# juniorliu95/replication_faster_rcnn

Measured on AMD Instinct MI355X. Metric: images/sec through RPN proposal+NMS+RoIPool; RoIPool HBM GB/s vs peak, higher is better.
Workload: dtype fp32; 1 GPU; cfg2: 8 images/GPU, VOC shape 600x1000, 38x63x9 anchors, 6000->300 NMS@0.7, RoIPool 7x7x256; global_batch=8, images_per_gpu=8, parallelism=dp1 (per-image sharding), streams=2, prop_streams=4, pool_on=prop, rng_waits=front, roi_cg=auto, roi_split=auto, roi_store=auto, prop_cus=0, devices=1, hw_queues=8

## Files before the change

### replication_faster_rcnn_amd/csrc/capi.cpp

```cpp
#include <hip/hip_runtime.h>

#include <cstdarg>
#include <cstdio>
#include <cstdlib>
#include <atomic>
#include <cstring>
#include <mutex>

#include "common.h"

namespace frcnn {

static thread_local char g_err[512] = "";
constexpr int kMaxDevices = 64;

void set_error(const char* fmt, ...) {
    va_list ap;
    va_start(ap, fmt);
    vsnprintf(g_err, sizeof(g_err), fmt, ap);
    va_end(ap);
}

int check_launch(const char* what) {
    hipError_t e = hipGetLastError();
    if (e != hipSuccess) {
        set_error("%s: %s", what, hipGetErrorString(e));
        return FRCNN_EHIP;
    }
    return FRCNN_OK;
}

static PathCfg g_path;

const PathCfg& path_cfg() { return g_path; }

int device_cu_count() {
    static std::atomic<int> cus[kMaxDevices] = {};
    int dev = 0;
    if (hipGetDevice(&dev) != hipSuccess || dev < 0 || dev >= kMaxDevices) {
        (void)hipGetLastError();
        return 256;
    }
    int n = cus[dev].load(std::memory_order_relaxed);
    if (n <= 0) {
        if (hipDeviceGetAttribute(&n, hipDeviceAttributeMultiprocessorCount, dev) != hipSuccess || n <= 0) {
            (void)hipGetLastError();
            n = 256;
        }
        cus[dev].store(n, std::memory_order_relaxed);
    }
    return n;
}

}

extern "C" const char* frcnn_version(void) { return "frcnn_mi355x 0.2.0 gfx950"; }

extern "C" int frcnn_set_path(const char* op, const char* path) {
    using namespace frcnn;
    if (!op || !path) {
        set_error("frcnn_set_path: null argument");
        return FRCNN_EINVAL;
    }
    auto is = [&](const char* a, const char* b) { return std::strcmp(a, b) == 0; };
    const bool aut = is(path, "auto");
    if (is(op, "roi_pool_fwd") &&
        (aut || is(path, "wave") || is(path, "dense") || is(path, "generic"))) {
        g_path.roi_fwd = aut ? kPathAuto : is(path, "generic") ? kPathGeneric
                                       : is(path, "dense")     ? kPathDense
                                                               : kPathWave;
    } else if (is(op, "roi_pool_bwd") &&
               (aut || is(path, "ring") || is(path, "plain"))) {
        g_path.roi_bwd = aut ? kPathAuto : is(path, "plain") ? kPathPlain : kPathRing;
    } else if (is(op, "propose") &&
               (aut || is(path, "hybrid") || is(path, "lazy") || is(path, "wide"))) {
        g_path.propose = aut ? kPathAuto : is(path, "hybrid") ? kPathHybrid
                                         : is(path, "lazy")   ? kPathLazy
                                                              : kPathWide;
    } else if (is(op, "roi_pool_fwd_store") && (aut || is(path, "temporal") || is(path, "nt"))) {
        g_path.roi_store = is(path, "nt") ? 1 : 0;
    } else if (is(op, "sampler") && (aut || is(path, "walk") || is(path, "chip") || is(path, "chip_only") ||
                                     is(path, "chip_tight"))) {
        g_path.sampler = aut                   ? kPathAuto
                         : is(path, "walk")      ? kPathWalk
                         : is(path, "chip")      ? kPathChip
                         : is(path, "chip_only") ? kPathChipOnly
                                                 : kPathChipTight;
    } else if (is(op, "roi_pool_split")) {
        char* end = nullptr;
        const long v = aut ? 0 : std::strtol(path, &end, 10);
        if (!aut && (end == path || *end != '\0' || v < 0 || v > 64)) {
            set_error("frcnn_set_path: roi_pool_split must be auto or 0..64, got '%s'", path);
            return FRCNN_EINVAL;
        }
        g_path.roi_split = static_cast<int>(v);
    } else if (is(op, "roi_pool_cg") && (aut || is(path, "4") || is(path, "8") || is(path, "16"))) {
        g_path.roi_cg = aut ? 0 : std::atoi(path);
    } else {
        set_error("frcnn_set_path: unknown op / path '%s' / '%s'", op, path);
        return FRCNN_EINVAL;
    }
    return FRCNN_OK;
}

extern "C" const char* frcnn_last_error(void) { return frcnn::g_err; }

extern "C" int frcnn_device_cu_count(int* out) {
    int dev = 0, n = 0;
    if (!out) {
        frcnn::set_error("frcnn_device_cu_count: null pointer");
        return FRCNN_EINVAL;
    }
    if (hipGetDevice(&dev) != hipSuccess ||
        hipDeviceGetAttribute(&n, hipDeviceAttributeMultiprocessorCount, dev) != hipSuccess)
        return frcnn::check_launch("frcnn_device_cu_count");
    *out = n;
    return FRCNN_OK;
}

extern "C" int frcnn_stream_create(const uint32_t* cu_mask, int words, void** out) {
    if (!out || words < 0 || (words > 0 && !cu_mask)) {
        frcnn::set_error("frcnn_stream_create: bad arguments");
        return FRCNN_EINVAL;
    }
    hipStream_t s = nullptr;
    const hipError_t e = words > 0 ? hipExtStreamCreateWithCUMask(&s, static_cast<uint32_t>(words), cu_mask)
                                   : hipStreamCreateWithFlags(&s, hipStreamNonBlocking);
    if (e != hipSuccess) {
        frcnn::set_error("frcnn_stream_create: %s", hipGetErrorString(e));
        return FRCNN_EHIP;
    }
    *out = s;
    return FRCNN_OK;
}

namespace frcnn {
struct CuCache {
    std::mutex mu;
    hipStream_t s[16] = {};
    int dev[16] = {};
    int n[16] = {};
    int next = 0;
};
static CuCache g_cu_cache;

static void cu_cache_evict(hipStream_t st) {
    std::lock_guard<std::mutex> lk(g_cu_cache.mu);
    for (int i = 0; i < 16; ++i)
        if (g_cu_cache.s[i] == st) g_cu_cache.s[i] = nullptr;
}
}

extern "C" int frcnn_stream_destroy(void* stream) {
    if (!stream) return FRCNN_OK;
    frcnn::cu_cache_evict(frcnn::as_stream(stream));
    if (hipStreamDestroy(frcnn::as_stream(stream)) != hipSuccess)
        return frcnn::check_launch("frcnn_stream_destroy");
    return FRCNN_OK;
}

namespace frcnn {
int stream_cu_count(hipStream_t s) {
    const int all = device_cu_count();
// ... 55 lines not shown
```

### replication_faster_rcnn_amd/csrc/common.h

```cpp
#pragma once

#include <hip/hip_runtime.h>

#include <cstdint>
#include <cstdio>
#include <string>

#include "../../include/frcnn_capi.h"

namespace frcnn {

void set_error(const char* fmt, ...);

constexpr int kPathAuto = 0;
constexpr int kPathGeneric = 1;
constexpr int kPathDense = 2;
constexpr int kPathWave = 3;
constexpr int kPathPlain = 1;
constexpr int kPathRing = 2;
constexpr int kPathHybrid = 1;
constexpr int kPathLazy = 2;
constexpr int kPathWide = 3;
constexpr int kPathWalk = 1;
constexpr int kPathChip = 2;
constexpr int kPathChipOnly = 3;
constexpr int kPathChipTight = 4;
struct PathCfg {
    int roi_fwd = kPathAuto;
    int roi_bwd = kPathAuto;
    int propose = kPathAuto;
    int roi_split = 0;
    int roi_cg = 0;
    int sampler = kPathAuto;
    int roi_store = 0;
};
const PathCfg& path_cfg();

int device_cu_count();
int stream_cu_count(hipStream_t s);

int check_launch(const char* what);

#define FRCNN_REQUIRE(cond, ...)                 \
    do {                                         \
        if (!(cond)) {                           \
            ::frcnn::set_error(__VA_ARGS__);     \
            return FRCNN_EINVAL;                 \
        }                                        \
    } while (0)

#define FRCNN_LAUNCH_CHECK(name)                         \
    do {                                                 \
        int _rc = ::frcnn::check_launch(name);           \
        if (_rc) return _rc;                             \
    } while (0)

inline hipStream_t as_stream(void* s) { return reinterpret_cast<hipStream_t>(s); }

inline size_t align_up(size_t x, size_t a) { return (x + a - 1) / a * a; }

struct Carver {
    char* base;
    size_t off = 0;
    explicit Carver(void* p) : base(static_cast<char*>(p)) {}
    template <class T>
    T* take(size_t count) {
        off = align_up(off, 256);
        T* p = reinterpret_cast<T*>(base ? base + off : nullptr);
        off += count * sizeof(T);
        return p;
    }
    size_t used() const { return align_up(off, 256); }
};

constexpr int kWave = 64;

__device__ __forceinline__ int lane_id() { return __lane_id(); }

__device__ __forceinline__ uint64_t readlane_u64(uint64_t v, int l) {
    uint32_t lo = __builtin_amdgcn_readlane(static_cast<uint32_t>(v), l);
    uint32_t hi = __builtin_amdgcn_readlane(static_cast<uint32_t>(v >> 32), l);
    return (static_cast<uint64_t>(hi) << 32) | lo;
}

__device__ __forceinline__ uint64_t wave_or_u64(uint64_t v) {
    for (int o = 32; o > 0; o >>= 1) v |= __shfl_xor(v, o, 64);
    return v;
}

__device__ __forceinline__ uint32_t wave_sum_u32(uint32_t v) {
    for (int o = 32; o > 0; o >>= 1) v += __shfl_xor(v, o, 64);
    return v;
}

__device__ __forceinline__ uint64_t lanemask_lt() {
    int l = lane_id();
    return l == 0 ? 0ull : (~0ull >> (64 - l));
}

__device__ __forceinline__ uint32_t desc_score_key(float s) {
    if (s != s) return 0u;
    uint32_t u = __float_as_uint(s);
    if (u == 0x80000000u) u = 0u;
    uint32_t asc = (u & 0x80000000u) ? ~u : (u | 0x80000000u);
    return ~asc;
}

__device__ __forceinline__ float clamp_nan(float v, float lo, float hi) {
    if (v != v) return v;
    float t = v < lo ? lo : v;
    return t > hi ? hi : t;
}

__device__ __forceinline__ float exp_cr(float v) { return static_cast<float>(exp(static_cast<double>(v))); }

__device__ __forceinline__ float4 decode_box(float4 a, float4 d) {
    float ah = a.z - a.x;
// ... 15 lines not shown
```

### replication_faster_rcnn_amd/csrc/roi_pool.hip

```cpp
#include <cfloat>
#include <cmath>
#include <cstdlib>
#include <cstring>

#include <type_traits>

#include <hip/hip_bf16.h>
#include <hip/hip_fp16.h>

#include "common.h"

namespace frcnn {

__device__ __forceinline__ float ld_f32(const float* p) { return *p; }
__device__ __forceinline__ float ld_f32(const __half* p) { return __half2float(*p); }
__device__ __forceinline__ float ld_f32(const __hip_bfloat16* p) { return __bfloat162float(*p); }
__device__ __forceinline__ __half cvt_elem(float v, const __half*) { return __float2half(v); }
__device__ __forceinline__ __hip_bfloat16 cvt_elem(float v, const __hip_bfloat16*) { return __float2bfloat16(v); }
__device__ __forceinline__ void st_f32(float* p, float v) { *p = v; }
template <class T>
__device__ __forceinline__ void st_f32(T* p, float v) {
    *p = cvt_elem(v, p);
}
__device__ __forceinline__ void st4_f32(float* p, float a, float b, float c, float d) {
    *reinterpret_cast<float4*>(p) = make_float4(a, b, c, d);
}
template <class T>
__device__ __forceinline__ void st4_f32(T* p, float a, float b, float c, float d) {
    struct alignas(8) Quad {
        T v[4];
    };
    static_assert(sizeof(Quad) == sizeof(uint2), "16-bit element types only");
    const Quad q{{cvt_elem(a, p), cvt_elem(b, p), cvt_elem(c, p), cvt_elem(d, p)}};
    *reinterpret_cast<uint2*>(p) = __builtin_bit_cast(uint2, q);
}
__device__ __forceinline__ void st_nt_f32(float* p, float v) { __builtin_nontemporal_store(v, p); }
template <class T>
__device__ __forceinline__ void st_nt_f32(T* p, float v) {
    static_assert(sizeof(T) == 2, "16-bit element types only");
    __builtin_nontemporal_store(__builtin_bit_cast(uint16_t, cvt_elem(v, p)), reinterpret_cast<uint16_t*>(p));
}

constexpr int kMaxBins = 1024;
constexpr int kListPad = 16;
__host__ __device__ constexpr int64_t list_stride(int64_t R) { return R + kListPad; }
constexpr size_t kLdsPerCu = 160 * 1024;

__device__ __forceinline__ int4 roi_bin(const float* roi, float ss, int H, int W, int PH, int PW,
                                        int ph, int pw) {
    int sw = static_cast<int>(roundf(roi[1] * ss));
    int sh = static_cast<int>(roundf(roi[2] * ss));
    int ew = static_cast<int>(roundf(roi[3] * ss));
    int eh = static_cast<int>(roundf(roi[4] * ss));
    int rw = ew - sw + 1;
    int rh = eh - sh + 1;
    rw = rw > 1 ? rw : 1;
    rh = rh > 1 ? rh : 1;
    float bh = static_cast<float>(rh) / static_cast<float>(PH);
    float bw = static_cast<float>(rw) / static_cast<float>(PW);
    int hs = static_cast<int>(floorf(static_cast<float>(ph) * bh)) + sh;
    int ws = static_cast<int>(floorf(static_cast<float>(pw) * bw)) + sw;
    int he = static_cast<int>(ceilf(static_cast<float>(ph + 1) * bh)) + sh;
    int we = static_cast<int>(ceilf(static_cast<float>(pw + 1) * bw)) + sw;
    hs = min(max(hs, 0), H);
    he = min(max(he, 0), H);
    ws = min(max(ws, 0), W);
    we = min(max(we, 0), W);
    return make_int4(hs, he, ws, we);
}

template <class T>
__device__ __forceinline__ void pool_window(const T* __restrict__ plane, int W, int4 g,
                                            float& mv, int& mi) {
    mv = (g.y <= g.x || g.w <= g.z) ? 0.0f : -FLT_MAX;
    mi = -1;
    for (int h = g.x; h < g.y; ++h) {
        const T* row = plane + h * W;
        for (int w = g.z; w < g.w; ++w) {
            float v = ld_f32(&row[w]);
            if (v > mv) {
                mv = v;
                mi = h * W + w;
            }
// ... 420 lines not shown
                const size_t o = (static_cast<size_t>(r) * C + c0) * PHW + k;
#pragma unroll
                for (int c = 0; c < CG; ++c) {
                    const int idx = mi[c] >> 4;
                    float v = mv[c];
                    if (v == 0.0f && idx >= 0)
                        v = reinterpret_cast<const float*>(tb + (c >> 2) * plane_bytes)[idx * 4 + (c & 3)];
                    st_f32(&out[o + static_cast<size_t>(c) * PHW], v);
                    argmax[o + static_cast<size_t>(c) * PHW] = idx;
                }
            }
            f0 = __builtin_amdgcn_readfirstlane(fn);
        }
    }
}

template <int NT, int CG, int FIX, bool HEAD, bool LIST>
__global__ __launch_bounds__(NT) void roi_pool_fwd_dense_kernel(
    const float* __restrict__ x, const float* __restrict__ rois, const int* __restrict__ list,
    const int* __restrict__ cnt, int R, int C, int H, int W, int PH_, int PW_, float ss,
    float* __restrict__ out, int32_t* __restrict__ argmax, int cap, HeadArgs hd) {
    roi_pool_fwd_dense_body<float, NT, CG, FIX, HEAD, LIST>(x, rois, list, cnt, R, C, H, W, PH_, PW_, ss, out,
                                                            argmax, cap, hd);
}

template <class T, int NT, int CG, int FIX, bool HEAD, bool LIST>
__global__ __launch_bounds__(NT) void roi_pool_fwd_dense_kernel_h(
    const T* __restrict__ x, const float* __restrict__ rois, const int* __restrict__ list,
    const int* __restrict__ cnt, int R, int C, int H, int W, int PH_, int PW_, float ss,
    T* __restrict__ out, int32_t* __restrict__ argmax, int cap, HeadArgs hd) {
    roi_pool_fwd_dense_body<T, NT, CG, FIX, HEAD, LIST>(x, rois, list, cnt, R, C, H, W, PH_, PW_, ss, out, argmax,
                                                        cap, hd);
}

#ifdef FRCNN_POOL_PROF
constexpr int kPoolProfSlots = 8192;
__device__ unsigned long long g_pool_prof[kPoolProfSlots][4];
__device__ unsigned int g_pool_prof_rois[kPoolProfSlots];
#define PPROF_T(k)                                                                                  \
    do {                                                                                            \
        const unsigned long long _t = __builtin_amdgcn_s_memrealtime();                             \
        const unsigned _wg = blockIdx.x + gridDim.x * (blockIdx.y + gridDim.y * blockIdx.z);         \
        if (_wg < kPoolProfSlots) {                                                                 \
            if ((k) == 3) {                                                                         \
                if ((threadIdx.x & 63) == 0) atomicMax(&g_pool_prof[_wg][3], _t);                   \
            } else if (threadIdx.x == 0) {                                                          \
                g_pool_prof[_wg][k] = _t;                                                           \
            }                                                                                       \
        }                                                                                           \
    } while (0)
#define PPROF_ROIS(n)                                                                               \
    do {                                                                                            \
        const unsigned _wg = blockIdx.x + gridDim.x * (blockIdx.y + gridDim.y * blockIdx.z);         \
        if (_wg < kPoolProfSlots && threadIdx.x == 0) g_pool_prof_rois[_wg] = (n);                  \
    } while (0)
#else
#define PPROF_T(k) do {} while (0)
#define PPROF_ROIS(n) do {} while (0)
#endif

constexpr int kFixPx = 2400;

typedef float f32x4 __attribute__((ext_vector_type(4)));
typedef __attribute__((address_space(3))) const f32x4 lds_f32x4;

template <int NP, int KPS>
__device__ __forceinline__ void tile_read(uint32_t a, uint32_t ps, f32x4 (&v)[NP]) {
    const uint32_t P = KPS ? static_cast<uint32_t>(KPS) : ps;
    uint32_t a2 = 0;
    if (NP > 2) {
        if (KPS) asm("v_add_u32_e32 %0, %1, %2" : "=v"(a2) : "i"(2 * KPS), "v"(a));
        else a2 = a + 2 * P;
    }
#pragma unroll
    for (int q = 0; q < NP; ++q) {
        const uint32_t o = q < 2 ? a + q * P : a2 + (q - 2) * P;
        v[q] = *reinterpret_cast<lds_f32x4*>(static_cast<size_t>(o));
    }
}

template <class T, int NT, int CG, int FIX, bool HEAD, bool NTS, int KPS>
__device__ __forceinline__ void roi_pool_fwd_wave_body(
    const T* x, const float* rois, int R, int C, int H, int W, int PH_, int PW_,
    float ss, T* out, int32_t* argmax, int geo_cap, HeadArgs hd) {
    const int PH = FIX ? FIX : PH_, PW = FIX ? FIX : PW_;
    constexpr int NP = CG / 4;
    extern __shared__ __attribute__((aligned(16))) float4 q4[];
    char* const t = reinterpret_cast<char*>(q4);
    if ((size_t)(__attribute__((address_space(3))) float4*)q4 != 0) __builtin_trap();
    const int b = blockIdx.z;
    const int c0 = blockIdx.x * CG;
    const int tid = threadIdx.x, lane = tid & 63;
    const int HW = H * W;
    const int HWs = (HW + 16) & ~15;
    const uint32_t PS = KPS ? static_cast<uint32_t>(KPS) : static_cast<uint32_t>(HWs) * 16u;
    int4* s_geo = reinterpret_cast<int4*>(t + NP * PS);
    int* s_red = reinterpret_cast<int*>(s_geo + geo_cap);
    int* s_next = s_red + 2 * (NT / 64);
    const int PHW = PH * PW;
    const int split = gridDim.y, z = blockIdx.y;
    const int N = gridDim.z - 1;
    PPROF_T(0);
    if (b == N) {
        const int2 rg = HEAD ? roi_range_sorted<NT>(hd.inds, R, 0, N, s_red, 1)
                             : roi_range_sorted<NT>(rois, R, 0, N, s_red);
        const int n_lo = rg.x, tot = n_lo + (R - rg.y);
        const int lo = static_cast<int>(static_cast<int64_t>(tot) * z / split);
        const int hi = static_cast<int>(static_cast<int64_t>(tot) * (z + 1) / split);
        if (HEAD && hd.boxes && blockIdx.x == 0)
            for (int t = lo + tid; t < hi; t += NT) {
                const int r = t < n_lo ? t : rg.y + (t - n_lo);
                float bx[5];
                head_box(rois, hd, r, bx);
#pragma unroll
                for (int j = 0; j < 5; ++j) hd.boxes[static_cast<size_t>(r) * 5 + j] = bx[j];
            }
        for (int e = lo * CG * PHW + tid; e < hi * CG * PHW; e += NT) {
            const int t = e / (CG * PHW);
            const int rem = e - t * (CG * PHW);
            const int r = t < n_lo ? t : rg.y + (t - n_lo);
            const size_t o = (static_cast<size_t>(r) * C + c0) * PHW + rem;
            st_f32(&out[o], 0.0f);
            argmax[o] = -1;
        }
        return;
    }
    const int2 rg = HEAD ? roi_range_sorted<NT>(hd.inds, R, b, b + 1, s_red, 1)
                         : roi_range_sorted<NT>(rois, R, b, b + 1, s_red);
    const int rbase = rg.x, nr = rg.y - rg.x;
    PPROF_T(1);
    if (z >= nr) return;
    const int nmine = (nr - z + split - 1) / split;
    PPROF_ROIS(nmine);
    const T* src = x + (static_cast<size_t>(b) * C + c0) * HW;
    if (tid < NP) *reinterpret_cast<float4*>(t + tid * PS + HW * 16) = make_float4(0.f, 0.f, 0.f, 0.f);
    for (int p = tid; p < HW; p += NT) {
        float v[CG];
#pragma unroll
        for (int q = 0; q < CG; ++q) {
            const float e = ld_f32(&src[static_cast<size_t>(q) * HW + p]);
            v[q] = e > -FLT_MAX ? e : -FLT_MAX;
        }
#pragma unroll
        for (int k = 0; k < NP; ++k)
            *reinterpret_cast<float4*>(t + k * PS + p * 16) = make_float4(v[4 * k], v[4 * k + 1], v[4 * k + 2], v[4 * k + 3]);
    }
    const int ph = lane / PW, pw = lane - (lane / PW) * PW;
    const bool act = lane < PHW;
    for (int k0 = 0; k0 < nmine; k0 += geo_cap) {
        const int cn = min(geo_cap, nmine - k0);
        for (int i = tid; i < cn; i += NT) {
            const int r = rbase + z + (k0 + i) * split;
            float bx[5];
            if (HEAD) {
                head_box(rois, hd, r, bx);
                if (hd.boxes && blockIdx.x == 0) {
#pragma unroll
                    for (int j = 0; j < 5; ++j) hd.boxes[static_cast<size_t>(r) * 5 + j] = bx[j];
                }
            } else {
#pragma unroll
                for (int j = 0; j < 5; ++j) bx[j] = rois[static_cast<size_t>(r) * 5 + j];
            }
            const RoiGeom gm = roi_geom(bx, ss, PH, PW);
            s_geo[i] = make_int4(gm.sh, gm.sw, __float_as_int(gm.bh), __float_as_int(gm.bw));
        }
        if (tid == 0) *s_next = 0;
        __syncthreads();
        if (k0 == 0) PPROF_T(2);
        int k = 0;
        if (lane == 0) k = atomicAdd(s_next, 1);
        k = __builtin_amdgcn_readfirstlane(k);
        while (k < cn) {
            int kn = 0;
            if (lane == 0) kn = atomicAdd(s_next, 1);
            const int r = rbase + z + (k0 + k) * split;
            const int4 gq = s_geo[k];
            RoiGeom gm;
            gm.sh = gq.x;
            gm.sw = gq.y;
            gm.bh = __int_as_float(gq.z);
            gm.bw = __int_as_float(gq.w);
            int4 g = geom_bin(gm, H, W, ph, pw);
            if (!act) g = make_int4(0, 0, 0, 0);
            const bool empty = g.y <= g.x || g.w <= g.z;
            float mv[CG];
            int mi[CG];
            {
                const uint32_t a0 = static_cast<uint32_t>(empty ? HW : g.x * W + g.z) * 16u;
                const float thr = empty ? __int_as_float(0x7f800000) : -FLT_MAX;
                f32x4 v[NP];
                tile_read<NP, KPS>(a0, PS, v);
                __builtin_amdgcn_sched_barrier(0);
#pragma unroll
                for (int q = 0; q < NP; ++q) {
                    const float vv[4] = {v[q].x, v[q].y, v[q].z, v[q].w};
#pragma unroll
                    for (int j = 0; j < 4; ++j) {
                        mv[4 * q + j] = vv[j];
                        mi[4 * q + j] = vv[j] > thr ? static_cast<int>(a0) : -1;
                    }
                }
            }
            for (int h = g.x; h < g.y; ++h) {
                const uint32_t rb = static_cast<uint32_t>(h * W) * 16u;
                const uint32_t ae = rb + static_cast<uint32_t>(g.w) * 16u;
                uint32_t a = rb + static_cast<uint32_t>(h == g.x ? g.z + 1 : g.z) * 16u;
                for (; a < ae; a += 16) {
                    f32x4 v[NP];
                    tile_read<NP, KPS>(a, PS, v);
                    __builtin_amdgcn_sched_barrier(0);
#pragma unroll
                    for (int q = 0; q < NP; ++q) {
                        const float vv[4] = {v[q].x, v[q].y, v[q].z, v[q].w};
#pragma unroll
                        for (int j = 0; j < 4; ++j) {
                            if (vv[j] > mv[4 * q + j]) {
                                mv[4 * q + j] = vv[j];
                                mi[4 * q + j] = static_cast<int>(a);
                            }
                        }
                    }
                }
            }
            if (act) {
                const size_t o = (static_cast<size_t>(r) * C + c0) * PHW + lane;
                T* op = out + o;
                int32_t* ap = argmax + o;
                if constexpr (NTS) {
#pragma unroll
                    for (int c = 0; c < CG; ++c) {
                        st_nt_f32(&op[c * PHW], mv[c]);
                        __builtin_nontemporal_store(mi[c] >> 4, ap + c * PHW);
                    }
                } else {
#pragma unroll
                    for (int c = 0; c < CG; ++c) {
                        st_f32(&op[c * PHW], mv[c]);
                        ap[c * PHW] = mi[c] >> 4;
                    }
                }
            }
            k = __builtin_amdgcn_readfirstlane(kn);
        }
        __syncthreads();
    }
    PPROF_T(3);
}

template <int NT, int CG, int FIX, bool HEAD, bool NTS = false, int KPS = 0>
__global__ __launch_bounds__(NT) void roi_pool_fwd_wave_kernel(
    const float* __restrict__ x, const float* __restrict__ rois, int R, int C, int H, int W, int PH_, int PW_,
    float ss, float* __restrict__ out, int32_t* __restrict__ argmax, int geo_cap, HeadArgs hd) {
    roi_pool_fwd_wave_body<float, NT, CG, FIX, HEAD, NTS, KPS>(x, rois, R, C, H, W, PH_, PW_, ss, out, argmax,
                                                               geo_cap, hd);
}

template <class T, int NT, int CG, int FIX, bool HEAD, bool NTS = false, int KPS = 0>
__global__ __launch_bounds__(NT) void roi_pool_fwd_wave_kernel_h(
    const T* __restrict__ x, const float* __restrict__ rois, int R, int C, int H, int W, int PH_, int PW_,
    float ss, T* __restrict__ out, int32_t* __restrict__ argmax, int geo_cap, HeadArgs hd) {
    roi_pool_fwd_wave_body<T, NT, CG, FIX, HEAD, NTS, KPS>(x, rois, R, C, H, W, PH_, PW_, ss, out, argmax, geo_cap,
                                                           hd);
}

__global__ __launch_bounds__(256) void roi_transform_kernel(const float* __restrict__ rois,
                                                            const float* __restrict__ inds,
                                                            int64_t R, float img_h, float img_w,
                                                            float fh, float fw,
                                                            float* __restrict__ boxes) {
    int64_t r = static_cast<int64_t>(blockIdx.x) * 256 + threadIdx.x;
    if (r >= R) return;
    float4 v = reinterpret_cast<const float4*>(rois)[r];
    float* o = boxes + r * 5;
    o[0] = inds[r];
    o[1] = v.x / img_h * fh;
    o[2] = v.y / img_w * fw;
    o[3] = v.z / img_h * fh;
    o[4] = v.w / img_w * fw;
}

template <class Flag>
__device__ __forceinline__ void roi_lists_image(const float* __restrict__ rois, int R, int N, int b,
                                                int* __restrict__ list, int* __restrict__ cnt, int stride,
                                                Flag flag_of) {
    const int tid = threadIdx.x, lane = tid & 63, wid = tid >> 6;
    __shared__ int s_w[16];
    __shared__ int s_last;
    int base = 0;
    for (int r0 = 0; r0 < R; r0 += 1024) {
        int r = r0 + tid;
        int rb = r < R ? static_cast<int>(rois[static_cast<size_t>(r) * stride]) : -1;
        bool m = r < R && (b < N ? rb == b : (rb < 0 || rb >= N));
        uint64_t bal = __ballot(m);
        if (lane == 0) s_w[wid] = __popcll(bal);
        __syncthreads();
        int before = 0, tot = 0;
        for (int w = 0; w < 16; ++w) {
            before += w < wid ? s_w[w] : 0;
            tot += s_w[w];
        }
        if (m) {
            const int flag = flag_of(r) ? static_cast<int>(0x80000000u) : 0;
            const int pos = base + before + __popcll(bal & lanemask_lt());
            list[static_cast<size_t>(b) * list_stride(R) + pos] = r | flag;
            if (pos == base + tot - 1) s_last = r | flag;
        }
        base += tot;
        __syncthreads();
    }
    if (tid == 0) cnt[b] = base;
    if (tid < kListPad) list[static_cast<size_t>(b) * list_stride(R) + base + tid] = base > 0 ? s_last : 0;
}

__global__ __launch_bounds__(1024) void roi_lists_kernel(const float* __restrict__ rois, int R,
                                                         int N, int* __restrict__ list,
                                                         int* __restrict__ cnt, int stride = 5,
                                                         const uint8_t* __restrict__ code = nullptr,
                                                         int PHW = 0) {
    roi_lists_image(rois, R, N, blockIdx.x, list, cnt, stride,
                    [&](int r) { return code && (code[static_cast<size_t>(r) * PHW] & 16); });
}

template <class T>
__device__ __forceinline__ void roi_pool_invalid_fill_body(const int* list,
                                                           const int* cnt,
                                                           int R, int N, size_t per_roi,
                                                           T* out,
                                                           int32_t* argmax,
                                                           const float* rois4,
                                                           HeadArgs hd) {
    const int n = cnt[N];
    for (int t = blockIdx.x; t < n; t += gridDim.x) {
        const int r = list[static_cast<size_t>(N) * list_stride(R) + t];
        const size_t base = static_cast<size_t>(r) * per_roi;
        if (hd.inds && threadIdx.x == 0) {
            float bx[5];
            head_box(rois4, hd, r, bx);
#pragma unroll
            for (int j = 0; j < 5; ++j) hd.boxes[static_cast<size_t>(r) * 5 + j] = bx[j];
        }
        for (size_t e = threadIdx.x; e < per_roi; e += 256) {
            st_f32(&out[base + e], 0.0f);
            argmax[base + e] = -1;
        }
    }
// ... 634 lines not shown
        g_bwd_prof[gw][3] = nr;
        g_bwd_prof[gw][4] = t_start;
        g_bwd_prof[gw][5] = t_end;
        g_bwd_prof[gw][6] = tq[0];
        g_bwd_prof[gw][7] = tq[1];
    }
#endif
}

template <int D, int PWT, int PHT>
__global__ __launch_bounds__(1024) void roi_pool_bwd_lead_kernel(
    const float* __restrict__ grad, const int32_t* __restrict__ argmax,
    const int* __restrict__ list, const int* __restrict__ cnt,
    int R, int C, int HW, int HWs, int PH_, int CPW, float* __restrict__ grad_in) {
    roi_pool_bwd_lead_body<float, D, PWT, PHT>(grad, argmax, list, cnt, R, C, HW, HWs, PH_, CPW, grad_in);
}

template <class T, int D, int PWT, int PHT>
__global__ __launch_bounds__(1024) void roi_pool_bwd_lead_kernel_h(
    const T* __restrict__ grad, const int32_t* __restrict__ argmax,
    const int* __restrict__ list, const int* __restrict__ cnt,
    int R, int C, int HW, int HWs, int PH_, int CPW, T* __restrict__ grad_in) {
    roi_pool_bwd_lead_body<T, D, PWT, PHT>(grad, argmax, list, cnt, R, C, HW, HWs, PH_, CPW, grad_in);
}

}

using namespace frcnn;

extern "C" int frcnn_roi_transform(const float* rois, const float* roi_inds, int64_t R, float img_h,
                                   float img_w, int feat_h, int feat_w, float* boxes,
                                   void* stream) {
    FRCNN_REQUIRE(R >= 0, "frcnn_roi_transform: R < 0");
    if (R == 0) return FRCNN_OK;
    FRCNN_REQUIRE(rois && roi_inds && boxes, "frcnn_roi_transform: null pointer");
    hipLaunchKernelGGL(roi_transform_kernel, dim3(static_cast<unsigned>((R + 255) / 256)),
                       dim3(256), 0, as_stream(stream), rois, roi_inds, R, img_h, img_w,
                       static_cast<float>(feat_h), static_cast<float>(feat_w), boxes);
    FRCNN_LAUNCH_CHECK("roi_transform_kernel");
    return FRCNN_OK;
}

#ifdef FRCNN_BWD_PROF
extern "C" int frcnn_debug_bwd_prof(unsigned long long* out, int reset) {
    (void)hipMemcpyFromSymbol(out, HIP_SYMBOL(g_bwd_prof), sizeof(g_bwd_prof));
    if (reset) {
        static unsigned long long z[kBwdProfWaves][8];
        (void)hipMemcpyToSymbol(HIP_SYMBOL(g_bwd_prof), z, sizeof(z));
    }
    return 0;
}
#endif
#ifdef FRCNN_POOL_PROF
extern "C" int frcnn_debug_pool_prof(unsigned long long* times, unsigned* rois, int reset) {
    (void)hipMemcpyFromSymbol(times, HIP_SYMBOL(g_pool_prof), sizeof(g_pool_prof));
    (void)hipMemcpyFromSymbol(rois, HIP_SYMBOL(g_pool_prof_rois), sizeof(g_pool_prof_rois));
    if (reset) {
        static unsigned long long zt[kPoolProfSlots][4];
        static unsigned zr[kPoolProfSlots];
        (void)hipMemcpyToSymbol(HIP_SYMBOL(g_pool_prof), zt, sizeof(zt));
        (void)hipMemcpyToSymbol(HIP_SYMBOL(g_pool_prof_rois), zr, sizeof(zr));
    }
    return 0;
}
#endif

namespace {
struct FwdWs {
    int* list;
    int* cnt;
    size_t bytes;
};
FwdWs carve_fwd(void* ws, int64_t R, int N) {
    Carver c(ws);
    FwdWs w{};
    w.list = c.take<int>(static_cast<size_t>(N + 1) * list_stride(R));
    w.cnt = c.take<int>(N + 1);
    w.bytes = c.used();
    return w;
}

struct PxPlan {
    int cg = 0, geo_cap = 0, split = 1;
    bool kps = false;
    size_t lds = 0;
};
constexpr size_t kWaveScratch = 256;
constexpr size_t kGeoCap = 368;
PxPlan px_plan(int C, int N, int H, int W, int PH, int PW, hipStream_t st, size_t per_geo = sizeof(int4)) {
    PxPlan pl;
    const size_t HW = static_cast<size_t>(H) * W;
    const int PHW = PH * PW;
    if (N <= 0 || HW == 0 || PHW > 64 || H > 65535 || W > 65535) return pl;
    constexpr size_t kReserve = 1024;
    const size_t kMinGeo = 64 * per_geo;
    const size_t HWs = (HW + 16) & ~static_cast<size_t>(15);
    auto fits = [&](size_t tile) {
        if (2 * (tile + kMinGeo + kWaveScratch + kReserve) <= kLdsPerCu) return 2;
        return tile + kMinGeo + kWaveScratch + kReserve <= kLdsPerCu ? 1 : 0;
    };
    for (int cg : {16, 8, 4}) {
        if (C % cg != 0) continue;
        if (path_cfg().roi_cg && cg != path_cfg().roi_cg) continue;
        const size_t tile_rt = static_cast<size_t>(cg / 4) * HWs * sizeof(float4);
        const bool kps = cg == 16 && PH == 7 && PW == 7 && HWs <= static_cast<size_t>(kFixPx) && fits(tile_rt) == 1;
        const size_t tile = kps ? static_cast<size_t>(cg / 4) * kFixPx * sizeof(float4) : tile_rt;
        const int per_cu = fits(tile);
        if (!per_cu) continue;
        const size_t geo = (kLdsPerCu / per_cu - kReserve - kWaveScratch - tile) / per_geo;
        pl.geo_cap = static_cast<int>(geo > kGeoCap ? kGeoCap : geo);
        pl.cg = cg;
        pl.kps = kps;
        pl.lds = tile + static_cast<size_t>(pl.geo_cap) * per_geo + kWaveScratch;
        const int64_t wgs = static_cast<int64_t>(C / cg) * N;
        int64_t sp = (static_cast<int64_t>(stream_cu_count(st)) * per_cu + wgs - 1) / wgs;
        if (path_cfg().roi_split > 0) sp = path_cfg().roi_split;
        pl.split = static_cast<int>(sp < 1 ? 1 : (sp > 64 ? 64 : sp));
        return pl;
    }
    return pl;
}

constexpr int kF32 = FRCNN_F32, kF16 = FRCNN_F16, kBF16 = FRCNN_BF16;
template <class T>
constexpr bool is_f32 = std::is_same_v<T, float>;

template <class T, bool HEAD>
int px_launch(const PxPlan& pl, const T* x, const float* rois, int64_t R, int N, int C, int H, int W,
              int PH, int PW, float ss, T* out, int32_t* argmax, const HeadArgs& hd, hipStream_t st) {
    const dim3 grid(static_cast<unsigned>(C / pl.cg), static_cast<unsigned>(pl.split), static_cast<unsigned>(N + 1));
    const bool fix7 = PH == 7 && PW == 7;
    FRCNN_REQUIRE(!pl.kps || fix7, "roi_pool_fwd: fixed-stride plan for a non-7x7 output");
#define FRCNN_PX_S(CG, FX, KP, NTSV)                                                                               \
    do {                                                                                                            \
        if constexpr (is_f32<T>)                                                                                    \
            hipLaunchKernelGGL((roi_pool_fwd_wave_kernel<1024, CG, FX, HEAD, NTSV, KP>), grid, dim3(1024), pl.lds,  \
                               st, x, rois, static_cast<int>(R), C, H, W, PH, PW, ss, out, argmax, pl.geo_cap, hd); \
        else                                                                                                        \
            hipLaunchKernelGGL((roi_pool_fwd_wave_kernel_h<T, 1024, CG, FX, HEAD, NTSV, KP>), grid, dim3(1024),     \
                               pl.lds, st, x, rois, static_cast<int>(R), C, H, W, PH, PW, ss, out, argmax,          \
                               pl.geo_cap, hd);                                                                     \
    } while (0)
#define FRCNN_PX(CG, FX, KP)                        \
    do {                                            \
        if (path_cfg().roi_store)                   \
            FRCNN_PX_S(CG, FX, KP, true);           \
        else                                        \
            FRCNN_PX_S(CG, FX, KP, false);          \
    } while (0)
    if (pl.cg == 16) {
        if (pl.kps) FRCNN_PX(16, 7, kFixPx * 16);
        else if (fix7) FRCNN_PX(16, 7, 0);
        else FRCNN_PX(16, 0, 0);
    } else if (pl.cg == 8) {
        if (fix7) FRCNN_PX(8, 7, 0); else FRCNN_PX(8, 0, 0);
    } else {
        if (fix7) FRCNN_PX(4, 7, 0); else FRCNN_PX(4, 0, 0);
    }
#undef FRCNN_PX
#undef FRCNN_PX_S
    FRCNN_LAUNCH_CHECK("roi_pool_fwd_wave_kernel");
    return FRCNN_OK;
}

struct DensePlan {
    int cg = 0, cap = 0, split = 1;
    size_t lds = 0;
};
DensePlan dense_plan(int C, int N, int H, int W, int PHW) {
    DensePlan pl;
    const size_t HW = static_cast<size_t>(H) * W;
    if (N <= 0 || HW == 0 || PHW > 64 || H > 65535 || W > 65535) return pl;
    const size_t HWs = (HW + 15) & ~static_cast<size_t>(15);
    const size_t fixed = dense_fixed_bytes() + 64;
    constexpr size_t kMinItems = 64;
    for (int cg : {16, 8, 4}) {
        if (C % cg != 0) continue;
        if (path_cfg().roi_cg && cg != path_cfg().roi_cg) continue;
        const size_t tile = static_cast<size_t>(cg / 4) * HWs * sizeof(float4);
        const size_t need = tile + fixed + kMinItems * dense_item_bytes();
        if (HWs * 16 * (cg / 4) >= (1u << 31) || need > kLdsPerCu) continue;
        const int per_cu = 2 * need <= kLdsPerCu ? 2 : 1;
        size_t cap = (kLdsPerCu / per_cu - tile - fixed) / dense_item_bytes();
        cap = cap > 4096 ? 4096 : cap;
        pl.cg = cg;
        pl.cap = static_cast<int>(cap & ~static_cast<size_t>(15));
        pl.lds = tile + fixed + static_cast<size_t>(pl.cap) * dense_item_bytes();
        const int64_t wgs = static_cast<int64_t>(C / cg) * N;
        const int64_t target = static_cast<int64_t>(device_cu_count()) * per_cu;
        int64_t sp = (target + wgs - 1) / wgs;
        if (path_cfg().roi_split > 0) sp = path_cfg().roi_split;
        pl.split = static_cast<int>(sp < 1 ? 1 : (sp > 64 ? 64 : sp));
        return pl;
    }
    return pl;
}

template <class T, bool HEAD, bool LIST>
int dense_launch(const DensePlan& pl, const T* x, const float* rois, const int* list, const int* cnt,
                 int64_t R, int N, int C, int H, int W, int PH, int PW, float ss, T* out,
                 int32_t* argmax, const HeadArgs& hd, hipStream_t st) {
    const dim3 grid(static_cast<unsigned>(C / pl.cg), static_cast<unsigned>(pl.split),
                    static_cast<unsigned>(LIST ? N : N + 1));
    const bool fix7 = PH == 7 && PW == 7;
#define FRCNN_DENSE(CG, FX)                                                                                    \
    do {                                                                                                       \
        if constexpr (is_f32<T>)                                                                               \
            hipLaunchKernelGGL((roi_pool_fwd_dense_kernel<1024, CG, FX, HEAD, LIST>), grid, dim3(1024), pl.lds, \
                               st, x, rois, list, cnt, static_cast<int>(R), C, H, W, PH, PW, ss, out, argmax,  \
                               pl.cap, hd);                                                                    \
        else                                                                                                   \
            hipLaunchKernelGGL((roi_pool_fwd_dense_kernel_h<T, 1024, CG, FX, HEAD, LIST>), grid, dim3(1024),   \
                               pl.lds, st, x, rois, list, cnt, static_cast<int>(R), C, H, W, PH, PW, ss, out,  \
                               argmax, pl.cap, hd);                                                            \
    } while (0)
    if (pl.cg == 16) {
        if (fix7) FRCNN_DENSE(16, 7); else FRCNN_DENSE(16, 0);
    } else if (pl.cg == 8) {
        if (fix7) FRCNN_DENSE(8, 7); else FRCNN_DENSE(8, 0);
    } else {
        if (fix7) FRCNN_DENSE(4, 7); else FRCNN_DENSE(4, 0);
    }
#undef FRCNN_DENSE
    FRCNN_LAUNCH_CHECK("roi_pool_fwd_dense_kernel");
// ... 460 lines not shown
```

Measured before the change: 119,800 images/sec.

## Schedule heavy RoIs first in RoIPool wave kernel to balance wave work

Each RoI's bin footprint is estimated when its geometry is computed. Up to a capped number of heavy RoIs (large footprint) are placed first in an LDS order list, so the atomic work queue hands them out early and waves avoid a long tail. The roi rows for the first chunk are prefetched before the feature tile loads, and the next queue index is fetched before the output stores. The change costs an extra LDS order array, which shrinks geo_cap, plus an added barrier and ballot per chunk.

```diff
diff --git a/replication_faster_rcnn_amd/csrc/capi.cpp b/replication_faster_rcnn_amd/csrc/capi.cpp
--- a/replication_faster_rcnn_amd/csrc/capi.cpp
+++ b/replication_faster_rcnn_amd/csrc/capi.cpp
@@ -79,6 +79,16 @@
                                                               : kPathWide;
     } else if (is(op, "roi_pool_fwd_store") && (aut || is(path, "temporal") || is(path, "nt"))) {
         g_path.roi_store = is(path, "nt") ? 1 : 0;
+    } else if (is(op, "roi_pool_order") && (aut || is(path, "index") || std::strncmp(path, "heavy", 5) == 0)) {
+        int t = 0, m = 0;
+        if (path[0] == 'h' && path[5] != '\0' &&
+            (std::sscanf(path + 5, ":%d:%d", &t, &m) != 2 || t < 1 || m < 1 || m > 64)) {
+            set_error("frcnn_set_path: roi_pool_order is auto, index, heavy or heavy:T:M, got '%s'", path);
+            return FRCNN_EINVAL;
+        }
+        g_path.roi_order = aut ? kPathAuto : is(path, "index") ? kPathIndex : kPathHeavy;
+        g_path.roi_heavy_thr = t;
+        g_path.roi_heavy_per_wave = m;
     } else if (is(op, "sampler") && (aut || is(path, "walk") || is(path, "chip") || is(path, "chip_only") ||
                                      is(path, "chip_tight"))) {
         g_path.sampler = aut                   ? kPathAuto
diff --git a/replication_faster_rcnn_amd/csrc/common.h b/replication_faster_rcnn_amd/csrc/common.h
--- a/replication_faster_rcnn_amd/csrc/common.h
+++ b/replication_faster_rcnn_amd/csrc/common.h
@@ -25,6 +25,8 @@
 constexpr int kPathChip = 2;
 constexpr int kPathChipOnly = 3;
 constexpr int kPathChipTight = 4;
+constexpr int kPathIndex = 1;
+constexpr int kPathHeavy = 2;
 struct PathCfg {
     int roi_fwd = kPathAuto;
     int roi_bwd = kPathAuto;
@@ -33,6 +35,9 @@
     int roi_cg = 0;
     int sampler = kPathAuto;
     int roi_store = 0;
+    int roi_order = kPathAuto;
+    int roi_heavy_thr = 0;
+    int roi_heavy_per_wave = 0;
 };
 const PathCfg& path_cfg();
 
diff --git a/replication_faster_rcnn_amd/csrc/roi_pool.hip b/replication_faster_rcnn_amd/csrc/roi_pool.hip
--- a/replication_faster_rcnn_amd/csrc/roi_pool.hip
+++ b/replication_faster_rcnn_amd/csrc/roi_pool.hip
@@ -1,4 +1,5 @@
 #include <cfloat>
+#include <climits>
 #include <cmath>
 #include <cstdlib>
 #include <cstring>
@@ -585,7 +586,7 @@
 template <class T, int NT, int CG, int FIX, bool HEAD, bool NTS, int KPS>
 __device__ __forceinline__ void roi_pool_fwd_wave_body(
     const T* x, const float* rois, int R, int C, int H, int W, int PH_, int PW_,
-    float ss, T* out, int32_t* argmax, int geo_cap, HeadArgs hd) {
+    float ss, T* out, int32_t* argmax, int geo_cap, int heavy_thr, int heavy_max, int heavy_share, HeadArgs hd) {
     const int PH = FIX ? FIX : PH_, PW = FIX ? FIX : PW_;
     constexpr int NP = CG / 4;
     extern __shared__ __attribute__((aligned(16))) float4 q4[];
@@ -598,11 +599,13 @@
     const int HWs = (HW + 16) & ~15;
     const uint32_t PS = KPS ? static_cast<uint32_t>(KPS) : static_cast<uint32_t>(HWs) * 16u;
     int4* s_geo = reinterpret_cast<int4*>(t + NP * PS);
-    int* s_red = reinterpret_cast<int*>(s_geo + geo_cap);
+    uint16_t* s_ord = reinterpret_cast<uint16_t*>(s_geo + geo_cap);
+    int* s_red = reinterpret_cast<int*>(s_ord + geo_cap);
     int* s_next = s_red + 2 * (NT / 64);
     const int PHW = PH * PW;
     const int split = gridDim.y, z = blockIdx.y;
     const int N = gridDim.z - 1;
+    const int wid = tid >> 6;
     PPROF_T(0);
     if (b == N) {
         const int2 rg = HEAD ? roi_range_sorted<NT>(hd.inds, R, 0, N, s_red, 1)
@@ -635,7 +638,20 @@
     if (z >= nr) return;
     const int nmine = (nr - z + split - 1) / split;
     PPROF_ROIS(nmine);
+    const int hthr = nmine <= heavy_share ? heavy_thr : INT_MAX;
     const T* src = x + (static_cast<size_t>(b) * C + c0) * HW;
+    auto load_row = [&](int r, float (&raw)[5]) {
+        if (HEAD) {
+            const float4 v = reinterpret_cast<const float4*>(rois)[r];
+            raw[0] = hd.inds[r];
+            raw[1] = v.x, raw[2] = v.y, raw[3] = v.z, raw[4] = v.w;
+        } else {
+#pragma unroll
+            for (int j = 0; j < 5; ++j) raw[j] = rois[static_cast<size_t>(r) * 5 + j];
+        }
+    };
+    float row0[5] = {0.f, 0.f, 0.f, 0.f, 0.f};
+    if (tid < min(geo_cap, nmine)) load_row(rbase + z + tid * split, row0);
     if (tid < NP) *reinterpret_cast<float4*>(t + tid * PS + HW * 16) = make_float4(0.f, 0.f, 0.f, 0.f);
     for (int p = tid; p < HW; p += NT) {
         float v[CG];
@@ -652,33 +668,60 @@
     const bool act = lane < PHW;
     for (int k0 = 0; k0 < nmine; k0 += geo_cap) {
         const int cn = min(geo_cap, nmine - k0);
-        for (int i = tid; i < cn; i += NT) {
+        bool heavy = false;
+        if (tid < cn) {
+            const int i = tid;
             const int r = rbase + z + (k0 + i) * split;
             float bx[5];
+            if (k0 == 0) {
+#pragma unroll
+                for (int j = 0; j < 5; ++j) bx[j] = row0[j];
+            } else {
+                load_row(r, bx);
+            }
             if (HEAD) {
-                head_box(rois, hd, r, bx);
+                bx[1] = bx[1] / hd.img_h * hd.fh;
+                bx[2] = bx[2] / hd.img_w * hd.fw;
+                bx[3] = bx[3] / hd.img_h * hd.fh;
+                bx[4] = bx[4] / hd.img_w * hd.fw;
                 if (hd.boxes && blockIdx.x == 0) {
 #pragma unroll
                     for (int j = 0; j < 5; ++j) hd.boxes[static_cast<size_t>(r) * 5 + j] = bx[j];
                 }
-            } else {
-#pragma unroll
-                for (int j = 0; j < 5; ++j) bx[j] = rois[static_cast<size_t>(r) * 5 + j];
             }
             const RoiGeom gm = roi_geom(bx, ss, PH, PW);
             s_geo[i] = make_int4(gm.sh, gm.sw, __float_as_int(gm.bh), __float_as_int(gm.bw));
-        }
+            const float fh = floorf(gm.bh), fw = floorf(gm.bw);
+            const int mh = min(static_cast<int>(fh) + (gm.bh > fh ? 2 : 0), H);
+            const int mw = min(static_cast<int>(fw) + (gm.bw > fw ? 2 : 0), W);
+            heavy = mh * mw >= hthr;
+        }
+        const uint64_t hbal = __ballot(heavy);
+        if (lane == 0) s_red[wid] = __popcll(hbal);
         if (tid == 0) *s_next = 0;
+        __syncthreads();
+        if (tid < cn) {
+            int before = __popcll(hbal & lanemask_lt()), tot = 0;
+            for (int w = 0; w < (cn + 63) >> 6; ++w) {
+                const int n = s_red[w];
+                before += w < wid ? n : 0;
+                tot += n;
+            }
+            const int nh = min(tot, heavy_max);
+            const int pos = heavy && before < heavy_max ? before : nh + tid - min(before, heavy_max);
+            s_ord[pos] = static_cast<uint16_t>(tid);
+        }
         __syncthreads();
         if (k0 == 0) PPROF_T(2);
         int k = 0;
         if (lane == 0) k = atomicAdd(s_next, 1);
         k = __builtin_amdgcn_readfirstlane(k);
+        int it = __builtin_amdgcn_readfirstlane(s_ord[k < cn ? k : 0]);
         while (k < cn) {
             int kn = 0;
             if (lane == 0) kn = atomicAdd(s_next, 1);
-            const int r = rbase + z + (k0 + k) * split;
-            const int4 gq = s_geo[k];
+            const int r = rbase + z + (k0 + it) * split;
+            const int4 gq = s_geo[it];
             RoiGeom gm;
             gm.sh = gq.x;
             gm.sw = gq.y;
@@ -726,6 +769,8 @@
                     }
                 }
             }
+            k = __builtin_amdgcn_readfirstlane(kn);
+            it = __builtin_amdgcn_readfirstlane(s_ord[k < cn ? k : 0]);
             if (act) {
                 const size_t o = (static_cast<size_t>(r) * C + c0) * PHW + lane;
                 T* op = out + o;
@@ -744,7 +789,6 @@
                     }
                 }
             }
-            k = __builtin_amdgcn_readfirstlane(kn);
         }
         __syncthreads();
     }
@@ -754,17 +798,19 @@
 template <int NT, int CG, int FIX, bool HEAD, bool NTS = false, int KPS = 0>
 __global__ __launch_bounds__(NT) void roi_pool_fwd_wave_kernel(
     const float* __restrict__ x, const float* __restrict__ rois, int R, int C, int H, int W, int PH_, int PW_,
-    float ss, float* __restrict__ out, int32_t* __restrict__ argmax, int geo_cap, HeadArgs hd) {
+    float ss, float* __restrict__ out, int32_t* __restrict__ argmax, int geo_cap, int heavy_thr,
+    int heavy_max, int heavy_share, HeadArgs hd) {
     roi_pool_fwd_wave_body<float, NT, CG, FIX, HEAD, NTS, KPS>(x, rois, R, C, H, W, PH_, PW_, ss, out, argmax,
-                                                               geo_cap, hd);
+                                                               geo_cap, heavy_thr, heavy_max, heavy_share, hd);
 }
 
 template <class T, int NT, int CG, int FIX, bool HEAD, bool NTS = false, int KPS = 0>
 __global__ __launch_bounds__(NT) void roi_pool_fwd_wave_kernel_h(
     const T* __restrict__ x, const float* __restrict__ rois, int R, int C, int H, int W, int PH_, int PW_,
-    float ss, T* __restrict__ out, int32_t* __restrict__ argmax, int geo_cap, HeadArgs hd) {
+    float ss, T* __restrict__ out, int32_t* __restrict__ argmax, int geo_cap, int heavy_thr,
+    int heavy_max, int heavy_share, HeadArgs hd) {
     roi_pool_fwd_wave_body<T, NT, CG, FIX, HEAD, NTS, KPS>(x, rois, R, C, H, W, PH_, PW_, ss, out, argmax, geo_cap,
-                                                           hd);
+                                                           heavy_thr, heavy_max, heavy_share, hd);
 }
 
 __global__ __launch_bounds__(256) void roi_transform_kernel(const float* __restrict__ rois,
@@ -1565,12 +1611,17 @@
 
 struct PxPlan {
     int cg = 0, geo_cap = 0, split = 1;
+    int heavy_thr = INT_MAX, heavy_max = 0, heavy_share = 0;
     bool kps = false;
     size_t lds = 0;
 };
 constexpr size_t kWaveScratch = 256;
-constexpr size_t kGeoCap = 368;
-PxPlan px_plan(int C, int N, int H, int W, int PH, int PW, hipStream_t st, size_t per_geo = sizeof(int4)) {
+constexpr size_t kGeoCap = 320;
+constexpr int kHeavyThr = 32;
+constexpr int kHeavyPerWave = 1;
+constexpr int kHeavyShare = 192;
+PxPlan px_plan(int C, int N, int H, int W, int PH, int PW, hipStream_t st,
+               size_t per_geo = sizeof(int4) + sizeof(uint16_t)) {
     PxPlan pl;
     const size_t HW = static_cast<size_t>(H) * W;
     const int PHW = PH * PW;
@@ -1591,7 +1642,12 @@
         const int per_cu = fits(tile);
         if (!per_cu) continue;
         const size_t geo = (kLdsPerCu / per_cu - kReserve - kWaveScratch - tile) / per_geo;
-        pl.geo_cap = static_cast<int>(geo > kGeoCap ? kGeoCap : geo);
+        pl.geo_cap = static_cast<int>(geo > kGeoCap ? kGeoCap : geo) & ~1;
+        if (path_cfg().roi_order != kPathIndex) {
+            pl.heavy_thr = path_cfg().roi_heavy_thr > 0 ? path_cfg().roi_heavy_thr : kHeavyThr;
+            pl.heavy_max = 16 * (path_cfg().roi_heavy_per_wave > 0 ? path_cfg().roi_heavy_per_wave : kHeavyPerWave);
+            pl.heavy_share = path_cfg().roi_order == kPathHeavy ? INT_MAX : kHeavyShare;
+        }
         pl.cg = cg;
         pl.kps = kps;
         pl.lds = tile + static_cast<size_t>(pl.geo_cap) * per_geo + kWaveScratch;
@@ -1618,11 +1674,12 @@
     do {                                                                                                            \
         if constexpr (is_f32<T>)                                                                                    \
             hipLaunchKernelGGL((roi_pool_fwd_wave_kernel<1024, CG, FX, HEAD, NTSV, KP>), grid, dim3(1024), pl.lds,  \
-                               st, x, rois, static_cast<int>(R), C, H, W, PH, PW, ss, out, argmax, pl.geo_cap, hd); \
+                               st, x, rois, static_cast<int>(R), C, H, W, PH, PW, ss, out, argmax, pl.geo_cap,     \
+                               pl.heavy_thr, pl.heavy_max, pl.heavy_share, hd);                                     \
         else                                                                                                        \
             hipLaunchKernelGGL((roi_pool_fwd_wave_kernel_h<T, 1024, CG, FX, HEAD, NTSV, KP>), grid, dim3(1024),     \
                                pl.lds, st, x, rois, static_cast<int>(R), C, H, W, PH, PW, ss, out, argmax,          \
-                               pl.geo_cap, hd);                                                                     \
+                               pl.geo_cap, pl.heavy_thr, pl.heavy_max, pl.heavy_share, hd);                         \
     } while (0)
 #define FRCNN_PX(CG, FX, KP)                        \
     do {                                            \
```

Result: no change. 119,600 images/sec (median of 4 runs) (-0.1%).
